# OllieBoyne/sslap

Measured on AMD Instinct MI355X. Metric: Medges/s (bid-phase CSR nnz/s) + solve ms, N=200k d=0.1% sparse LAP, higher is better.
Workload: dtype f64

## Files before the change

sslap_amd/csrc/device_common.hpp:

```cpp
#pragma once
#include <hip/hip_runtime.h>
#include <stdint.h>

#include <type_traits>

namespace misslap {

constexpr int kWave = 64;
constexpr int kPosNone = 0x7fffffff;
constexpr int kTailMax = 512;

#define MISSLAP_KERNEL(BLOCK) MISSLAP_KERNEL_BOUND(BLOCK, BLOCK)
#define MISSLAP_KERNEL_BOUND(BLOCK, BOUND)                                                          \
    static constexpr int kBlock = (BLOCK);    \
    static constexpr int kBound = (BOUND);      \
    static_assert(kBlock <= kBound, "a launch above the kernel's bound fails");                     \
    template <class... A_>                                                                          \
    static __global__ __launch_bounds__(BOUND) void entry(A_... a_) {                               \
        run(a_...);                                                                                 \
    }

constexpr int kErrNegativeBid = 1;
constexpr int kErrRowsUnsorted = 2;
constexpr int kErrRowGap = 4;
// ... 142 lines not shown
};

constexpr int kDppXor1 = 0xB1;
constexpr int kDppXor2 = 0x4E;
constexpr int kDppHalfMirror = 0x141;
constexpr int kDppMirror = 0x140;
constexpr int kDppBcast15 = 0x142;
constexpr int kDppBcast31 = 0x143;
template <int CTRL, int ROW_MASK = 0xF>
__device__ __forceinline__ int dpp_i32(int v) {
    return __builtin_amdgcn_update_dpp(v, v, CTRL, ROW_MASK, 0xF, false);
}
template <int CTRL, int ROW_MASK = 0xF>
__device__ __forceinline__ double dpp_f64(double v) {
    const int lo = dpp_i32<CTRL, ROW_MASK>(__double2loint(v));
    const int hi = dpp_i32<CTRL, ROW_MASK>(__double2hiint(v));
    return __hiloint2double(hi, lo);
}
__device__ __forceinline__ double readlane_f64(double v, int l) {
    const int lo = __builtin_amdgcn_readlane(__double2loint(v), l);
    const int hi = __builtin_amdgcn_readlane(__double2hiint(v), l);
    return __hiloint2double(hi, lo);
}

#define MISSLAP_WAVE_MAX_STEP(T, EXCH) \
    {                                  \
        const T o = EXCH;              \
        v = o > v ? o : v;             \
    }
__device__ __forceinline__ int wave_max_i32(int v) {
    MISSLAP_WAVE_MAX_STEP(int, __builtin_amdgcn_mov_dpp(v, kDppXor1, 0xF, 0xF, true))
    MISSLAP_WAVE_MAX_STEP(int, __builtin_amdgcn_mov_dpp(v, kDppXor2, 0xF, 0xF, true))
    MISSLAP_WAVE_MAX_STEP(int, __builtin_amdgcn_mov_dpp(v, kDppHalfMirror, 0xF, 0xF, true))
    MISSLAP_WAVE_MAX_STEP(int, __builtin_amdgcn_mov_dpp(v, kDppMirror, 0xF, 0xF, true))
    MISSLAP_WAVE_MAX_STEP(int, (dpp_i32<kDppBcast15, 0xA>(v)))
    MISSLAP_WAVE_MAX_STEP(int, (dpp_i32<kDppBcast31, 0xC>(v)))
    return __builtin_amdgcn_readlane(v, 63);
}
__device__ __forceinline__ double wave_max_f64(double v) {
    v = __builtin_fmax(v, dpp_f64<kDppXor1>(v));
    v = __builtin_fmax(v, dpp_f64<kDppXor2>(v));
    v = __builtin_fmax(v, dpp_f64<kDppHalfMirror>(v));
    v = __builtin_fmax(v, dpp_f64<kDppMirror>(v));
    v = __builtin_fmax(v, (dpp_f64<kDppBcast15, 0xA>(v)));
    v = __builtin_fmax(v, (dpp_f64<kDppBcast31, 0xC>(v)));
    return readlane_f64(v, 63);
}
#undef MISSLAP_WAVE_MAX_STEP

struct Top2 {
    double v, w;
    int g;
};
__device__ __forceinline__ Top2 top2_wave_reduce(const Top2 &x) {
    Top2 r;
    r.v = wave_max_f64(x.v);
    r.g = wave_max_i32(x.v == r.v ? x.g : -1);
    r.w = wave_max_f64(x.g == r.g ? x.w : x.v);
    return r;
}

struct __attribute__((aligned(16))) PriceRec {
    double price;
    int owner;
    int ostart;
};

__device__ __forceinline__ int lane_id() { return threadIdx.x & (kWave - 1); }
__device__ __forceinline__ unsigned long long lanemask_lt() {
    return (1ull << lane_id()) - 1ull;
}

constexpr int kCandLanes = 32;
constexpr int kCandMax = 30;
constexpr int kCandMin = 24;
constexpr int kCandRowMax = 4 * kWave;

template <int CTRL>
__device__ __forceinline__ int dppf_i32(int v) {
    return __builtin_amdgcn_mov_dpp(v, CTRL, 0xF, 0xF, true);
}
template <int CTRL>
__device__ __forceinline__ double dppf_f64(double v) {
    return __hiloint2double(dppf_i32<CTRL>(__double2hiint(v)), dppf_i32<CTRL>(__double2loint(v)));
}
__device__ __forceinline__ double half_max_f64(double v) {
    v = __builtin_fmax(v, dppf_f64<kDppXor1>(v));
    v = __builtin_fmax(v, dppf_f64<kDppXor2>(v));
    v = __builtin_fmax(v, dppf_f64<kDppHalfMirror>(v));
    v = __builtin_fmax(v, dppf_f64<kDppMirror>(v));
    v = __builtin_fmax(v, (dpp_f64<kDppBcast15, 0xA>(v)));
    return v;
}
__device__ __forceinline__ int half_max_i32(int v) {
    v = max(v, dppf_i32<kDppXor1>(v));
    v = max(v, dppf_i32<kDppXor2>(v));
    v = max(v, dppf_i32<kDppHalfMirror>(v));
    v = max(v, dppf_i32<kDppMirror>(v));
    v = max(v, (dpp_i32<kDppBcast15, 0xA>(v)));
    return v;
}
__device__ __forceinline__ int half_allmax_i32(int v) {
    v = max(v, dppf_i32<kDppXor1>(v));
    v = max(v, dppf_i32<kDppXor2>(v));
    v = max(v, dppf_i32<kDppHalfMirror>(v));
    v = max(v, dppf_i32<kDppMirror>(v));
    const auto s = __builtin_amdgcn_permlane16_swap(v, v, false, false);
    return max((int)s[0], (int)s[1]);
}

__device__ __forceinline__ double slot_cost(const int2 &s) { return (double)__int_as_float(s.y); }
__device__ __forceinline__ double slot_cost(const Slot64 &s) { return s.c; }
__device__ __forceinline__ double slot_cost_at(const int2 &s, int sl) {
    return (double)__int_as_float(__builtin_amdgcn_readlane(s.y, sl));
}
__device__ __forceinline__ double slot_cost_at(const Slot64 &s, int sl) { return readlane_f64(s.c, sl); }
template <class Slot>
struct LineIO;
template <>
struct LineIO<int2> {
    static __device__ __forceinline__ int2 load(const int2 *cand, const double *, size_t idx) { return cand[idx]; }
    static __device__ __forceinline__ int2 make(int x, int y) { return make_int2(x, y); }
};
template <>
struct LineIO<Slot64> {
    static __device__ __forceinline__ Slot64 load(const int2 *cand, const double *cost, size_t idx) {
        const int2 s = cand[idx];
        Slot64 r;
        r.x = s.x;
        r.y = s.y;
        r.c = cost[idx];
        return r;
    }
    static __device__ __forceinline__ Slot64 make(int x, int y) {
        Slot64 r;
        r.x = x;
        r.y = y;
        r.c = 0.0;
        return r;
    }
};

struct CandBid {
    bool hit;
    unsigned long long key;
    int obj;
    int prev, pstart;
    int len;
};

struct RecSource {
    const PriceRec *rec;
    __device__ __forceinline__ PriceRec get(int col) const { return rec[col]; }
};
struct PriceSource {
    const double *price;
    __device__ __forceinline__ PriceRec get(int col) const {
        PriceRec r;
        r.price = price[col];
        r.owner = -1;
        r.ostart = 0;
        return r;
    }
};

template <class Slot, class Src>
__device__ __forceinline__ PriceRec cand_gather2(const Slot slot, const bool act0, const bool act1, const Src &src) {
    const int lane = lane_id(), l32 = lane & (kCandLanes - 1);
    const bool active = lane < kCandLanes ? act0 : act1;
    const bool is_cand = active & (l32 >= 1) & (l32 <= kCandMax) & (slot.x >= 0);
    return src.get(is_cand ? slot.x : 0);
}
template <class Slot, class Early, class S = NoStamp>
__device__ __forceinline__ void cand_eval2_r(Slot &slot, const PriceRec r, const bool act0, const bool act1,
                                             const double eps, CandBid (&out)[2], int &err, Early &&early,
                                             const S &stamp = S(), int *alive = nullptr);
template <class Slot, class Src, class Early, class S = NoStamp>
__device__ __forceinline__ void cand_eval2(Slot &slot, const bool act0, const bool act1, const Src &src,
                                           const double eps, CandBid (&out)[2], int &err, Early &&early,
                                           const S &stamp = S(), int *alive = nullptr) {
    stamp(1);
    const PriceRec r = cand_gather2(slot, act0, act1, src);
    stamp(2);
    cand_eval2_r(slot, r, act0, act1, eps, out, err, early, stamp, alive);
}
template <class Slot, class Early, class S>
__device__ __forceinline__ void cand_eval2_r(Slot &slot, const PriceRec r, const bool act0, const bool act1,
                                             const double eps, CandBid (&out)[2], int &err, Early &&early,
                                             const S &stamp, int *alive) {
    const int lane = lane_id(), l32 = lane & (kCandLanes - 1);
    const double ninf = -__builtin_huge_val();
    const bool active = lane < kCandLanes ? act0 : act1;
    const bool is_cand = active & (l32 >= 1) & (l32 <= kCandMax) & (slot.x >= 0);
    const double cost = slot_cost(slot);
    double tau[2];
    tau[0] = readlane_f64(__hiloint2double(slot.y, slot.x), 0);
    tau[1] = readlane_f64(__hiloint2double(slot.y, slot.x), kCandLanes);
    out[0].len = __builtin_amdgcn_readlane(slot.x, kCandLanes - 1);
    out[1].len = __builtin_amdgcn_readlane(slot.x, 2 * kCandLanes - 1);
    const double v = is_cand ? cost - r.price : ninf;
    if (alive) {
        const unsigned long long al = __ballot(is_cand & (v >= (lane < kCandLanes ? tau[0] : tau[1])));
        alive[0] = __popc((unsigned)al);
        alive[1] = __popc((unsigned)(al >> 32));
    }
    double V[2], W[2];
    int G[2];
    {
        const double vm = half_max_f64(v);
        V[0] = readlane_f64(vm, 31);
        V[1] = readlane_f64(vm, 63);
        const double Vv = lane < kCandLanes ? V[0] : V[1];
        const int gm = half_max_i32((is_cand & (v == Vv)) ? l32 : -1);
        G[0] = __builtin_amdgcn_readlane(gm, 31);
        G[1] = __builtin_amdgcn_readlane(gm, 63);
    }
    double c1[2];
#pragma unroll
    for (int X = 0; X < 2; ++X) {
        const int sl = kCandLanes * X + max(G[X], 0);
        out[X].obj = __builtin_amdgcn_readlane(slot.x, sl);
        out[X].prev = __builtin_amdgcn_readlane(r.owner, sl);
        out[X].pstart = __builtin_amdgcn_readlane(r.ostart, sl);
        c1[X] = slot_cost_at(slot, sl);
    }
    early(out);
    stamp.light(3);
    const int Gv = lane < kCandLanes ? G[0] : G[1];
    const double wm = half_max_f64(l32 == Gv ? ninf : v);
    W[0] = readlane_f64(wm, 31);
    W[1] = readlane_f64(wm, 63);
#pragma unroll
    for (int X = 0; X < 2; ++X) {
        out[X].hit = (G[X] >= 0) & (V[X] > tau[X]) & (W[X] >= tau[X]);
        const double bid = (c1[X] - W[X]) + eps;
        if (out[X].hit && bid_is_bad(bid)) err |= kErrNegativeBid;
        out[X].key = bid_to_key(bid);
    }
}
template <class Slot, class Src>
__device__ __forceinline__ PriceRec cand_gather1(const Slot &slot, const bool cls, const Src &src) {
    const bool is_cand = cls & (slot.x >= 0);
    return src.get(is_cand ? slot.x : 0);
}
template <class Slot, class Early, class S = NoStamp>
__device__ __forceinline__ void cand_eval1_r(Slot &slot, const PriceRec r, const bool cls, const double eps, CandBid &out,
                                             unsigned &bad_hi, Early &&early, const S &stamp = S());
template <class Slot, class Src, class Early, class S = NoStamp>
__device__ __forceinline__ void cand_eval1(Slot &slot, const bool cls, const Src &src, const double eps, CandBid &out,
                                           unsigned &bad_hi, Early &&early, const S &stamp = S()) {
    stamp(1);
    const PriceRec r = cand_gather1(slot, cls, src);
    stamp(2);
    cand_eval1_r(slot, r, cls, eps, out, bad_hi, early, stamp);
}
template <class Slot, class Early, class S>
__device__ __forceinline__ void cand_eval1_r(Slot &slot, const PriceRec r, const bool cls, const double eps, CandBid &out,
                                             unsigned &bad_hi, Early &&early, const S &stamp) {
    const int lane = lane_id();
    const double ninf = -__builtin_huge_val();
    const bool is_cand = cls & (slot.x >= 0);
    const double cost = slot_cost(slot);
    const double tau = readlane_f64(__hiloint2double(slot.y, slot.x), 0);
    out.len = __builtin_amdgcn_readlane(slot.x, kCandLanes - 1);
    const double v = is_cand ? cost - r.price : ninf;
    const int hi = __double2hiint(v);
    const int k = hi ^ ((hi >> 31) & 0x7fffffff);
    const int km = __builtin_amdgcn_readlane(half_max_i32(k), 31);
    const unsigned eq = (unsigned)(__ballot(k == km) & 0xffffffffull);
    double V;
    int G;
    if (__popc(eq) == 1) {
        G = __ffs((int)eq) - 1;
        V = readlane_f64(v, G);
    } else {
        V = readlane_f64(half_max_f64(v), 31);
        G = __builtin_amdgcn_readlane(half_max_i32((is_cand & (v == V)) ? lane : -1), 31);
    }
    const int sl = max(G, 0);
    out.obj = __builtin_amdgcn_readlane(slot.x, sl);
    out.prev = __builtin_amdgcn_readlane(r.owner, sl);
    out.pstart = __builtin_amdgcn_readlane(r.ostart, sl);
    const double c1 = slot_cost_at(slot, sl);
    early(out);
    stamp.light(3);
    const double W = readlane_f64(half_max_f64(lane == G ? ninf : v), 31);
    out.hit = (G >= 0) & (V > tau) & (W >= tau);
    const double bid = (c1 - W) + eps;
    bad_hi = max(bad_hi, out.hit ? (unsigned)__double2hiint(bid) : 0u);
    out.key = bid_to_key(bid);
}
__device__ __forceinline__ bool bad_hi_is_error(unsigned bad_hi) { return bad_hi > 0x7ff00000u; }
struct NoEarly {
    __device__ __forceinline__ void operator()(const CandBid (&)[2]) const {}
    __device__ __forceinline__ void operator()(const CandBid &) const {}
};

struct CandBuildArgs {
    int c[4];
    double a[4], v[4];
    double V, W;
    int len;
    bool want;
};

__device__ __forceinline__ void cand_build(int2 *cand, double *cost, int person, const CandBuildArgs &ba, double eps,
                                           double &hint) {
    const int lane = lane_id();
    const double ninf = -__builtin_huge_val();
    const int len = ba.len;
    const double W = ba.W;
    unsigned long long okm[4];
#pragma unroll
    for (int u = 0; u < 4; ++u) {
        const int rem = len - kWave * u;
        okm[u] = rem >= kWave ? ~0ull : (rem <= 0 ? 0ull : ((1ull << rem) - 1ull));
    }
    auto count = [&](double t) {
        int n = 0;
#pragma unroll
        for (int u = 0; u < 4; ++u) n += __popcll(__ballot(ba.v[u] >= t) & okm[u]);
        return n;
    };
    double t = ninf;
    int n = len;
    if (len > kCandMax) {
        n = count(W);
        if (n > kCandMax) return;
        t = W;
        double d_ok = 0.0, d_bad = __builtin_huge_val();
        double d = hint > 0.0 ? hint : 4.0 * __builtin_fmax(ba.V - W, eps);
        for (int k = 0; k < 40 && n < kCandMin; ++k) {
            const double t2 = W - d;
            const int n2 = count(t2);
            if (n2 <= kCandMax) {
                d_ok = d;
                t = t2;
                n = n2;
                d = d_bad == __builtin_huge_val() ? 2.0 * d : 0.5 * (d_ok + d_bad);
            } else {
                d_bad = d;
                d = 0.5 * (d_ok + d_bad);
            }
            if (!(d > d_ok) || !(d < d_bad)) break;
        }
        hint = d_ok > 0.0 ? d_ok : hint;
    }
    int2 *line = cand + (size_t)person * kCandLanes;
    int base = 0;
#pragma unroll
    for (int u = 0; u < 4; ++u) {
        const unsigned long long m = __ballot(ba.v[u] >= t) & okm[u];
        if ((m >> lane) & 1ull) {
            const int at = 1 + base + __popcll(m & lanemask_lt());
            line[at] = make_int2(ba.c[u], cost ? 0 : __float_as_int((float)ba.a[u]));
            if (cost) cost[(size_t)person * kCandLanes + at] = ba.a[u];
        }
        base += __popcll(m);
    }
    if (lane < kCandLanes && (lane == 0 || lane == kCandLanes - 1 || lane > n)) {
        int2 x = make_int2(-1, 0);
        if (lane == 0) x = make_int2(__double2loint(t), __double2hiint(t));
        if (lane == kCandLanes - 1) x = make_int2(len, 0);
        line[lane] = x;
    }
}

template <class E, class Src, bool kNT, bool kPre>
__device__ __forceinline__ void wave_bid_full(const E &ed, const Src &src, int s, int e_in,
                                              const typename E::Raw (&pre)[4], double eps, CandBid &out,
                                              CandBuildArgs &ba, int &err) {
    const int lane = lane_id();
    const double ninf = -__builtin_huge_val();
    Top2 x;
    x.v = ninf;
    x.w = ninf;
    x.g = -1;
    int c1 = 0, o1 = -1, os1 = 0;
    double a1 = 0.0;
    int c[4];
    double a[4];
    auto load = [&](int g, int &cc, double &aa) {
        if (kNT) ed.load_nt(g, cc, aa);
        else ed.load(g, cc, aa);
    };
#pragma unroll
    for (int u = 0; u < 4; ++u) {
        if (kPre) E::decode(pre[u], c[u], a[u]);
        else load(s + u * kWave + lane, c[u], a[u]);
    }
    const int e = __builtin_amdgcn_readfirstlane(e_in);
    auto chunk = [&](int base, auto first_) {
        constexpr bool kFirst = decltype(first_)::value;
        PriceRec r[4];
#pragma unroll
        for (int u = 0; u < 4; ++u) {
            const bool ok = base + u * kWave + lane < e;
            if (!ok) c[u] = -1;
            r[u] = src.get(ok ? c[u] : 0);
        }
#pragma unroll
        for (int u = 0; u < 4; ++u) {
            const bool ok = c[u] >= 0;
            const double v = ok ? a[u] - r[u].price : ninf;
            const bool ge = ok & (v >= x.v);
            x.w = __builtin_fmax(x.w, __builtin_fmin(v, x.v));
            x.v = __builtin_fmax(x.v, v);
            x.g = ge ? base + u * kWave + lane : x.g;
            c1 = ge ? c[u] : c1;
            a1 = ge ? a[u] : a1;
            o1 = ge ? r[u].owner : o1;
            os1 = ge ? r[u].ostart : os1;
            if (kFirst && E::kCand) {
                ba.c[u] = c[u];
                ba.a[u] = a[u];
                ba.v[u] = v;
            }
        }
    };
    chunk(s, std::true_type{});
    for (int base = s + 4 * kWave; base < e; base += 4 * kWave) {
#pragma unroll
        for (int u = 0; u < 4; ++u) load(min(base + u * kWave + lane, e - 1), c[u], a[u]);
        chunk(base, std::false_type{});
    }
    const int hi = __double2hiint(x.v);
    const int k = hi ^ ((hi >> 31) & 0x7fffffff);
    const int kmax = wave_max_i32(k);
    const unsigned long long cnd = __ballot(k == kmax);
    int sl;
    double W;
    if (__popcll(cnd) == 1) {
        sl = __ffsll((long long)cnd) - 1;
        W = wave_max_f64(lane == sl ? x.w : x.v);
    } else {
        const int g_mine = x.g;
        const Top2 t2 = top2_wave_reduce(x);
        sl = __ffsll((long long)__ballot(g_mine == t2.g)) - 1;
// ... 134 lines not shown
```

sslap_amd/csrc/kernels_tail.hpp:

```cpp
#pragma once
#include "device_common.hpp"

namespace misslap {

struct TailArgs {
    Ctl *ctl;
    const int *row_ptr;
    double *price;
    PriceRec *rec;
    int *p2o;
    int *o2p;
    int *U;
    int2 *cand;
    double *cand64;
    int thr;
    int round_budget;
    float eps;
};

constexpr int kHashSize = 2048;

__device__ __forceinline__ unsigned long long readlane_u64(unsigned long long v, int l) {
    const int lo = __builtin_amdgcn_readlane((int)(unsigned)(v & 0xffffffffull), l);
    const int hi = __builtin_amdgcn_readlane((int)(unsigned)(v >> 32), l);
    return ((unsigned long long)(unsigned)hi << 32) | (unsigned long long)(unsigned)lo;
}

__device__ __forceinline__ int apply_winner(const TailArgs &a, int person, int pstart, int obj, int prev,
                                            unsigned long long key) {
    PriceRec r;
    r.price = key_to_bid(key);
    r.owner = person;
    r.ostart = pstart;
    a.rec[obj] = r;
    return prev;
}

struct k_sync_from_rec {
    MISSLAP_KERNEL(256)
    static __device__ __forceinline__ void run(Ctl *ctl, const PriceRec *rec, double *price, int *o2p, int *p2o, const int *U, int n_cols, int lines, unsigned long long *live, unsigned ticket) {
        const int K = ctl->K;
        if (blockIdx.x == 0 && threadIdx.x == 0) {
            post_live_status(live, ticket, K, ctl->err, ctl->nits);
            ctl->n_need = 0;
        }
        for (int n = blockIdx.x * blockDim.x + threadIdx.x; n < K; n += gridDim.x * blockDim.x) {
            const int i = U[n];
            if (i >= 0) p2o[i] = -1;
        }
        for (int j = blockIdx.x * blockDim.x + threadIdx.x; j < n_cols; j += gridDim.x * blockDim.x) {
            const PriceRec r = rec[j];
            if (lines && r.price < price[j]) atomicOr(&ctl->err, kErrPriceFell);
            price[j] = r.price;
            o2p[j] = r.owner;
            if (r.owner >= 0) p2o[r.owner] = j;
        }
    }
};


struct TailStats {
    unsigned long long edges, miss_edges, builds;
    unsigned bids, misses;
    unsigned bad_hi;
    int err;
    double hint;
};

__device__ __forceinline__ int lane_zero() {
    return (int)__builtin_amdgcn_mbcnt_hi(0u, __builtin_amdgcn_mbcnt_lo(0u, 0u));
}

template <class Slot>
__device__ __forceinline__ Slot cand_no_line() {
    return (lane_id() & (kCandLanes - 1)) == 0 ? LineIO<Slot>::make(0, 0x7ff00000) : LineIO<Slot>::make(-1, 0);
}
template <class E>
__device__ __forceinline__ typename E::Slot line_of(const TailArgs &a, int p, int l32) {
    return LineIO<typename E::Slot>::load(a.cand, a.cand64, (size_t)max(p, 0) * kCandLanes + l32);
}
template <class E>
struct TwoFetch {
    typename E::Slot slot;
    typename E::Raw row[2][4];
    int ev[2];
};
template <class E>
__device__ __forceinline__ void fetch_row(const TailArgs &a, const E &ed, int person, int start,
                                          typename E::Raw (&row)[4], int &e) {
    const int lane = lane_id();
#pragma unroll
    for (int u = 0; u < 4; ++u) row[u] = ed.load_raw_nt(start + u * kWave + lane);
    e = a.row_ptr[max(person, 0) + 1 + lane_zero()];
}
template <class E>
__device__ __forceinline__ void request_two(const TailArgs &a, const E &ed, int p0, int s0, int p1, int s1,
                                            TwoFetch<E> &tf) {
    if (E::kCand) {
        const int pme = lane_id() < kCandLanes ? p0 : p1;
        tf.slot = a.cand != nullptr ? line_of<E>(a, pme, lane_id() & (kCandLanes - 1)) : cand_no_line<typename E::Slot>();
    } else {
        fetch_row<E>(a, ed, p0, s0, tf.row[0], tf.ev[0]);
        fetch_row<E>(a, ed, p1, s1, tf.row[1], tf.ev[1]);
    }
}

__device__ __forceinline__ void tail_build(const TailArgs &a, int person, const CandBuildArgs &ba, double eps,
                                           TailStats &st) {
    cand_build(a.cand, a.cand64, person, ba, eps, st.hint);
    st.builds += 1;
}

template <class E, class Early, class S = NoStamp>
__device__ __forceinline__ void bid_two(const TailArgs &a, const E &ed, const int (&pi)[2], const int (&ps)[2],
                                        TwoFetch<E> &tf, double eps, CandBid (&b)[2], CandBuildArgs &bd,
                                        int &bd_person, TailStats &st, Early &&early, const S &stamp = S()) {
    const RecSource src{a.rec};
    b[0].hit = b[1].hit = false;
    if (E::kCand) cand_eval2(tf.slot, pi[0] >= 0, pi[1] >= 0, src, eps, b, st.err, early, stamp);
    stamp.light(4);
    bd_person = -1;
#pragma unroll
    for (int X = 0; X < 2; ++X) {
        if (pi[X] < 0) continue;
        if (!b[X].hit) {
            if (bd_person >= 0) tail_build(a, bd_person, bd, eps, st);
            if (E::kCand) {
                const typename E::Raw none[4] = {};
                const int e = a.row_ptr[pi[X] + 1 + lane_zero()];
                wave_bid_full<E, RecSource, true, false>(ed, src, ps[X], e, none, eps, b[X], bd, st.err);
            } else {
                wave_bid_full<E, RecSource, true, true>(ed, src, ps[X], tf.ev[X], tf.row[X], eps, b[X], bd, st.err);
            }
            bd.want = bd.want && a.cand != nullptr;
            bd_person = bd.want ? pi[X] : -1;
            st.misses += 1;
            st.miss_edges += (unsigned long long)b[X].len;
        }
        st.edges += (unsigned long long)b[X].len;
        st.bids += 1;
    }
}

__device__ __forceinline__ int round_limit(long long nits, long long max_iter) {
    return (int)min(max_iter - nits, (long long)0x7fffffff);
}

template <class E>
__device__ __forceinline__ void tail_chain_mode(const TailArgs &a, const E &ed, int &pi, int &ps, int &K,
                                                long long &nits, const long long max_iter, const double eps,
                                                TailStats &st) {
    const int lane = lane_id(), l32 = lane & (kCandLanes - 1);
    const RecSource src{a.rec};
    const bool cls = (lane >= 1) & (lane <= kCandMax);
    const bool lines = E::kCand && a.cand != nullptr;
    typename E::Slot slot = cand_no_line<typename E::Slot>();
    typename E::Raw row[4];
    int ev = 0;
    auto request = [&](int person, int start) {
        if (E::kCand) {
            if (lines) slot = line_of<E>(a, person, l32);
        } else {
            fetch_row<E>(a, ed, person, start, row, ev);
        }
    };
    request(pi, ps);
    const int rmax = round_limit(nits, max_iter);
    int r = 0;
#ifdef MISSLAP_TAIL_STAMP
    unsigned long long sacc[8] = {0, 0, 0, 0, 0, 0, 0, 0}, sprev = __builtin_amdgcn_s_memtime();
    const CycleStamp stamp{sacc, &sprev, true};
#else
    const NoStamp stamp;
#endif
    for (;;) {
        CandBid b;
        b.hit = false;
        int sp = -2;
        if (E::kCand)
            cand_eval1(slot, cls, src, eps, b, st.bad_hi, [&](const CandBid &w) {
                sp = w.prev;
                request(sp, 0);
            }, stamp);
        stamp.light(4);
        if (!b.hit) {
            CandBuildArgs bd;
            if (E::kCand) {
                const typename E::Raw none[4] = {};
                const int e = a.row_ptr[pi + 1];
                wave_bid_full<E, RecSource, true, false>(ed, src, ps, e, none, eps, b, bd, st.err);
            } else {
                wave_bid_full<E, RecSource, true, true>(ed, src, ps, ev, row, eps, b, bd, st.err);
            }
            st.misses += 1;
            st.miss_edges += (unsigned long long)b.len;
            if (bd.want && lines) tail_build(a, pi, bd, eps, st);
        }
        stamp.light(5);
        st.edges += (unsigned long long)b.len;
        st.bids += 1;
        r += 1;
        if (lane == 0) apply_winner(a, pi, ps, b.obj, b.prev, b.key);
        pi = b.prev;
        ps = b.pstart;
        const bool done = pi < 0 || r >= rmax;
        if (!done && sp != pi) request(pi, ps);
        stamp.light(6);
        if (done) break;
    }
    K = pi != -1;
    nits += r;
#ifdef MISSLAP_TAIL_STAMP
    if (lane == 0) {
        for (int k = 1; k <= 6; ++k) a.ctl->dbg[5 + k] += sacc[k];
    }
#endif
}

template <class E>
__device__ __forceinline__ void tail_solo_mode(const TailArgs &a, const E &ed, int *sU, int *sStart, int &K,
                                               long long &nits, const long long max_iter, const double eps,
                                               TailStats &st) {
    const int lane = lane_id();
    int pi[2], ps[2];
    pi[0] = __builtin_amdgcn_readfirstlane(sU[0]);
    ps[0] = __builtin_amdgcn_readfirstlane(sStart[0]);
    pi[1] = K > 1 ? __builtin_amdgcn_readfirstlane(sU[1]) : -1;
    ps[1] = K > 1 ? __builtin_amdgcn_readfirstlane(sStart[1]) : 0;
    if (K == 1) {
        tail_chain_mode(a, ed, pi[0], ps[0], K, nits, max_iter, eps, st);
        if (lane == 0) {
            sU[0] = pi[0];
            sU[1] = -1;
            sStart[0] = ps[0];
        }
        return;
    }
    TwoFetch<E> tf;
    tf.slot = cand_no_line<typename E::Slot>();
    request_two(a, ed, pi[0], ps[0], pi[1], ps[1], tf);
#ifdef MISSLAP_TAIL_STAMP_SOLO
    unsigned long long sacc[8] = {0, 0, 0, 0, 0, 0, 0, 0}, sprev = __builtin_amdgcn_s_memtime();
    const CycleStamp stamp{sacc, &sprev, true};
#else
    const NoStamp stamp;
#endif
    for (;;) {
        CandBid b[2];
        CandBuildArgs bd;
        int bd_person;
        int sp[2] = {-2, -2};
        bid_two(a, ed, pi, ps, tf, eps, b, bd, bd_person, st, [&](const CandBid(&w)[2]) {
            sp[0] = pi[0] >= 0 ? w[0].prev : -1;
            sp[1] = pi[1] >= 0 ? w[1].prev : -1;
            request_two(a, ed, sp[0], 0, sp[1], 0, tf);
        }, stamp);
        stamp.light(5);
        nits += 1;
        bool win0 = true, win1 = pi[1] >= 0;
        if (win1 && b[0].obj == b[1].obj) {
            if (b[1].key > b[0].key) win0 = false;
            else win1 = false;
        }
        if (lane == 0) {
            if (win0) apply_winner(a, pi[0], ps[0], b[0].obj, b[0].prev, b[0].key);
            if (win1) apply_winner(a, pi[1], ps[1], b[1].obj, b[1].prev, b[1].key);
        }
        if (win0) {
            pi[0] = b[0].prev;
            ps[0] = b[0].pstart;
        }
        if (win1) {
            pi[1] = b[1].prev;
            ps[1] = b[1].pstart;
        }
        if (pi[0] == -1 && pi[1] != -1) {
            pi[0] = pi[1];
            ps[0] = ps[1];
            pi[1] = -1;
        }
        K = (pi[0] != -1) + (pi[1] != -1);
        const bool done = K <= 1 || nits >= max_iter;
        if (!done && (sp[0] != pi[0] || sp[1] != pi[1])) request_two(a, ed, pi[0], ps[0], pi[1], ps[1], tf);
        if (bd_person >= 0) tail_build(a, bd_person, bd, eps, st);
        stamp.light(6);
        if (done) break;
    }
    if (K == 1 && nits < max_iter) tail_chain_mode(a, ed, pi[0], ps[0], K, nits, max_iter, eps, st);
#ifdef MISSLAP_TAIL_STAMP_SOLO
    if (lane == 0)
        for (int k = 1; k <= 6; ++k) a.ctl->dbg[5 + k] += sacc[k];
#endif
    if (lane == 0) {
        sU[0] = pi[0];
        sU[1] = pi[1];
        sStart[0] = ps[0];
        sStart[1] = ps[1];
    }
}

template <class E>
__device__ __forceinline__ void tail_pair_mode(const TailArgs &a, const E &ed, int *sU, int *sStart, int &K,
                                               long long &nits, const long long max_iter, const double eps,
                                               TailStats &st) {
    const int lane = lane_id(), l32 = lane & (kCandLanes - 1);
    const bool upper = lane >= kCandLanes;
    const RecSource src{a.rec};
    const bool cls = (l32 >= 1) & (l32 <= kCandMax);
    const double ninf = -__builtin_huge_val();
    int pi[2], ps[2];
#pragma unroll
    for (int X = 0; X < 2; ++X) {
        pi[X] = __builtin_amdgcn_readfirstlane(sU[X]);
        ps[X] = __builtin_amdgcn_readfirstlane(sStart[X]);
    }
    typename E::Slot slot;
    auto request = [&](int p0, int p1) { slot = line_of<E>(a, upper ? p1 : p0, l32); };
    const int rmax = round_limit(nits, max_iter);
    int r = 0;
    if (K == 2) request(pi[0], pi[1]);
#ifdef MISSLAP_TAIL_STAMP_DUO
    unsigned long long sacc[8] = {0, 0, 0, 0, 0, 0, 0, 0}, sprev = __builtin_amdgcn_s_memtime();
    const CycleStamp stamp{sacc, &sprev, true};
#else
    const NoStamp stamp;
#endif
    while (K == 2) {
        stamp(1);
        const PriceRec g = cand_gather1(slot, cls, src);
        stamp(2);
        const bool is_cand = cls & (slot.x >= 0);
        const double v = is_cand ? slot_cost(slot) - g.price : ninf;
        const int hw = __double2hiint(v);
        const int k = hw ^ ((hw >> 31) & 0x7fffffff);
        const unsigned long long eq = __ballot(k == half_allmax_i32(k));
        const unsigned eq0 = (unsigned)eq, eq1 = (unsigned)(eq >> 32);
        int G[2];
        double V[2];
        if ((int)(__popc(eq0) == 1) & (int)(__popc(eq1) == 1)) {
            G[0] = __ffs((int)eq0) - 1;
            G[1] = __ffs((int)eq1) + (kCandLanes - 1);
            V[0] = readlane_f64(v, G[0]);
            V[1] = readlane_f64(v, G[1]);
        } else {
            const double vm = half_max_f64(v);
            V[0] = readlane_f64(vm, kCandLanes - 1);
            V[1] = readlane_f64(vm, kWave - 1);
            const int gm = half_max_i32((is_cand & (v == (upper ? V[1] : V[0]))) ? lane : -1);
            G[0] = __builtin_amdgcn_readlane(gm, kCandLanes - 1);
            G[1] = __builtin_amdgcn_readlane(gm, kWave - 1);
        }
        CandBid b[2];
        double tau[2], c1[2];
#pragma unroll
        for (int X = 0; X < 2; ++X) {
            const int sl = max(G[X], kCandLanes * X);
            tau[X] = readlane_f64(__hiloint2double(slot.y, slot.x), kCandLanes * X);
            b[X].len = __builtin_amdgcn_readlane(slot.x, kCandLanes * X + kCandLanes - 1);
            b[X].obj = __builtin_amdgcn_readlane(slot.x, sl);
            b[X].prev = __builtin_amdgcn_readlane(g.owner, sl);
            b[X].pstart = __builtin_amdgcn_readlane(g.ostart, sl);
            c1[X] = slot_cost_at(slot, sl);
        }
        const int sp0 = b[0].prev, sp1 = b[1].prev;
        request(sp0, sp1);
        stamp.light(3);
        const double wm = half_max_f64(((lane == G[0]) | (lane == G[1])) ? ninf : v);
        const double W[2] = {readlane_f64(wm, kCandLanes - 1), readlane_f64(wm, kWave - 1)};
#pragma unroll
        for (int X = 0; X < 2; ++X) {
            b[X].hit = (G[X] >= 0) & (V[X] > tau[X]) & (W[X] >= tau[X]);
            const double bid = (c1[X] - W[X]) + eps;
            st.bad_hi = max(st.bad_hi, b[X].hit ? (unsigned)__double2hiint(bid) : 0u);
            b[X].key = bid_to_key(bid);
        }
        stamp.light(4);
#pragma unroll
        for (int X = 0; X < 2; ++X) {
            if (!b[X].hit) {
                CandBuildArgs bd;
                const typename E::Raw none[4] = {};
                const int e = a.row_ptr[pi[X] + 1];
                wave_bid_full<E, RecSource, true, false>(ed, src, ps[X], e, none, eps, b[X], bd, st.err);
                st.misses += 1;
                st.miss_edges += (unsigned long long)b[X].len;
                if (bd.want) tail_build(a, pi[X], bd, eps, st);
            }
        }
        stamp.light(5);
        st.edges += (unsigned long long)(b[0].len + b[1].len);
        st.bids += 2;
        r += 1;
        if ((b[0].obj != b[1].obj) & (b[0].prev >= 0) & (b[1].prev >= 0)) {
            if (l32 == 0) {
                PriceRec w;
                w.price = key_to_bid(upper ? b[1].key : b[0].key);
                w.owner = upper ? pi[1] : pi[0];
                w.ostart = upper ? ps[1] : ps[0];
                a.rec[upper ? b[1].obj : b[0].obj] = w;
            }
#pragma unroll
            for (int X = 0; X < 2; ++X) {
                pi[X] = b[X].prev;
                ps[X] = b[X].pstart;
            }
        } else {
            bool win0 = true, win1 = true;
            if (b[0].obj == b[1].obj) {
                if (b[1].key > b[0].key) win0 = false;
                else win1 = false;
            }
            if (lane == 0) {
                if (win0) apply_winner(a, pi[0], ps[0], b[0].obj, b[0].prev, b[0].key);
                if (win1) apply_winner(a, pi[1], ps[1], b[1].obj, b[1].prev, b[1].key);
            }
            if (win0) {
                pi[0] = b[0].prev;
                ps[0] = b[0].pstart;
            }
            if (win1) {
                pi[1] = b[1].prev;
                ps[1] = b[1].pstart;
            }
            if (pi[0] == -1 && pi[1] != -1) {
                pi[0] = pi[1];
                ps[0] = ps[1];
                pi[1] = -1;
            }
            K = (pi[0] != -1) + (pi[1] != -1);
        }
        const bool done = K <= 1 || r >= rmax;
        if (!done && (sp0 != pi[0] || sp1 != pi[1])) request(pi[0], pi[1]);
        stamp.light(6);
        if (done) break;
    }
    nits += r;
#ifdef MISSLAP_TAIL_STAMP_DUO
    if (lane == 0)
        for (int k = 1; k <= 6; ++k) a.ctl->dbg[5 + k] += sacc[k];
#endif
    if (K == 1 && nits < max_iter) tail_chain_mode(a, ed, pi[0], ps[0], K, nits, max_iter, eps, st);
    if (lane == 0) {
        sU[0] = pi[0];
        sU[1] = pi[1];
        sStart[0] = ps[0];
        sStart[1] = ps[1];
    }
}

constexpr int kTeamMax = 16;
constexpr int kTeamTab = 64;
__device__ __forceinline__ void tail_barrier_lds() { asm volatile("s_waitcnt lgkmcnt(0)\n\ts_barrier" ::: "memory"); }

template <class E>
__device__ __forceinline__ void tail_team_mode(const TailArgs &a, const E &ed, int *sU, int *sStart, int &K,
                                               long long &nits, const long long max_iter, const double eps,
                                               TailStats &st) {
    const int lane = lane_id(), wave = __builtin_amdgcn_readfirstlane(threadIdx.x >> 6);
    static_assert(kTeamMax <= 2 * (kTailMax / kWave) && kTeamMax <= kWave, "two list slots per wavefront");
    __shared__ unsigned long long tKey[2][kTeamMax];
    __shared__ int tObj[2][kTeamMax], tPrev[2][kTeamMax], tPst[2][kTeamMax], tU[2][kTeamMax], tS[2][kTeamMax];
    __shared__ int wTab[kTailMax / kWave][kTeamTab];
    const int n0 = 2 * wave;
    int pi[2], ps[2];
#pragma unroll
    for (int X = 0; X < 2; ++X) {
        pi[X] = n0 + X < K ? __builtin_amdgcn_readfirstlane(sU[min(n0 + X, kTailMax - 1)]) : -1;
        ps[X] = n0 + X < K ? __builtin_amdgcn_readfirstlane(sStart[min(n0 + X, kTailMax - 1)]) : 0;
    }
    wTab[wave][lane & (kTeamTab - 1)] = -1;
    TwoFetch<E> tf;
    tf.slot = cand_no_line<typename E::Slot>();
    if (n0 < K) request_two(a, ed, pi[0], ps[0], pi[1], ps[1], tf);
    __syncthreads();
#ifdef MISSLAP_TAIL_STAMP_TEAM
    unsigned long long sacc[8] = {0, 0, 0, 0, 0, 0, 0, 0}, sprev = __builtin_amdgcn_s_memtime();
    const CycleStamp stamp{sacc, &sprev, wave == 0};
#else
    const NoStamp stamp;
#endif
    int par = 0;
    for (;;) {
        int sp[2] = {-2, -2};
        CandBuildArgs bd;
        int bd_person = -1;
        stamp.light(0);
        if (n0 < K) {
            CandBid b[2];
            bid_two(a, ed, pi, ps, tf, eps, b, bd, bd_person, st, [&](const CandBid(&w)[2]) {
                sp[0] = pi[0] >= 0 ? w[0].prev : -1;
                sp[1] = pi[1] >= 0 ? w[1].prev : -1;
                request_two(a, ed, sp[0], 0, sp[1], 0, tf);
            });
            if (lane == 0) {
#pragma unroll
                for (int X = 0; X < 2; ++X)
                    if (pi[X] >= 0) {
                        tKey[par][n0 + X] = b[X].key;
                        tObj[par][n0 + X] = b[X].obj;
                        tPrev[par][n0 + X] = b[X].prev;
                        tPst[par][n0 + X] = b[X].pstart;
                        tU[par][n0 + X] = pi[X];
                        tS[par][n0 + X] = ps[X];
                    }
            }
        }
        stamp.light(1);
        tail_barrier_lds();
        stamp.light(2);
        {
            const bool act = lane < K;
            const int ls = min(lane, kTeamMax - 1);
            const unsigned long long lkey = act ? tKey[par][ls] : 0ull;
            const int lobj = act ? tObj[par][ls] : (-2 - lane);
            const int lprev = act ? tPrev[par][ls] : 0, lpst = act ? tPst[par][ls] : 0;
            int u = act ? tU[par][ls] : -1;
            int sx = act ? tS[par][ls] : 0;
            int hs = 0;
            bool dup = false;
            if (act) {
                hs = (int)(((unsigned)lobj * 2654435761u) >> 26) & (kTeamTab - 1);
                for (;;) {
                    const int old = atomicCAS(&wTab[wave][hs], -1, lobj);
                    if (old == -1) break;
                    if (old == lobj) {
                        dup = true;
                        break;
                    }
                    hs = (hs + 1) & (kTeamTab - 1);
                }
            }
            const bool contested = __any(dup);
            if (act && !dup) wTab[wave][hs] = -1;
            const bool ends = __any(act && lprev == -1);
#ifdef MISSLAP_TAIL_STAMP_TEAM
            if (threadIdx.x == 0) sacc[5] += (!contested && !ends), sacc[6] += contested, sacc[7] += 1;
#endif
            if (!contested && !ends) {
                if (act && n0 < K) apply_winner(a, u, sx, lobj, lprev, lkey);
#pragma unroll
                for (int X = 0; X < 2; ++X) {
                    const int w = __builtin_amdgcn_readlane(lprev, min(n0 + X, kWave - 1));
                    const int ws = __builtin_amdgcn_readlane(lpst, min(n0 + X, kWave - 1));
                    pi[X] = n0 + X < K ? w : -1;
                    ps[X] = n0 + X < K ? ws : 0;
                }
            } else {
                bool lose = false;
                for (int m = 0; m < K; ++m) {
                    const int om = __builtin_amdgcn_readlane(lobj, m);
                    const bool same = (om == lobj) && (m != lane);
                    if (__any(same)) {
                        const unsigned long long km = readlane_u64(lkey, m);
                        lose |= same && (km > lkey || (km == lkey && m < lane));
                    }
                }
                const bool won = act && !lose;
                if (won && n0 < K) apply_winner(a, u, sx, lobj, lprev, lkey);
                u = won ? lprev : u;
                sx = won ? lpst : sx;
                const unsigned long long kmask = (1ull << K) - 1ull;
                const unsigned long long holes = __ballot(act && u == -1) & kmask;
                const int Kn = K - __popcll(holes);
                const unsigned long long lmask = (1ull << Kn) - 1ull;
                unsigned long long hl = holes & lmask;
                unsigned long long mv = ~holes & ~lmask & kmask;
                while (hl) {
                    const int hk = __ffsll((long long)hl) - 1, mk = __ffsll((long long)mv) - 1;
                    const int mu = __builtin_amdgcn_readlane(u, mk), ms = __builtin_amdgcn_readlane(sx, mk);
                    if (lane == hk) {
                        u = mu;
                        sx = ms;
                    }
                    hl &= hl - 1;
                    mv &= mv - 1;
                }
                K = Kn;
#pragma unroll
                for (int X = 0; X < 2; ++X) {
                    pi[X] = n0 + X < K ? __builtin_amdgcn_readlane(u, min(n0 + X, kWave - 1)) : -1;
                    ps[X] = n0 + X < K ? __builtin_amdgcn_readlane(sx, min(n0 + X, kWave - 1)) : 0;
                }
            }
        }
        stamp.light(3);
        par ^= 1;
        nits += 1;
// ... 578 lines not shown
```

Baseline: 4831.

## Issue next candidate-line prefetch from high-word argmax and double-buffer tail slots

In the single-chain and duo tail loops, the owner of the best candidate is now found from the high 32 bits of the bid value alone. That lets the next person's candidate line be requested before the full f64 argmax and second-best reductions run. Candidate slots are double-buffered (slotA/slotB, with the loop unrolled by two) so the prefetch writes a separate register set while the current one is still in use. The gather now uses an unsigned, masked index, and sched_barriers pin the ordering. The prefetch is speculative: on a high-word tie or a mismatch the line is fetched again, which costs an extra load and adds register pressure.

```diff
diff --git a/sslap_amd/csrc/device_common.hpp b/sslap_amd/csrc/device_common.hpp
--- a/sslap_amd/csrc/device_common.hpp
+++ b/sslap_amd/csrc/device_common.hpp
@@ -318,6 +318,7 @@
 struct RecSource {
     const PriceRec *rec;
     __device__ __forceinline__ PriceRec get(int col) const { return rec[col]; }
+    __device__ __forceinline__ PriceRec get_u(unsigned col) const { return rec[(size_t)col]; }
 };
 struct PriceSource {
     const double *price;
@@ -412,14 +413,6 @@
 template <class Slot, class Early, class S = NoStamp>
 __device__ __forceinline__ void cand_eval1_r(Slot &slot, const PriceRec r, const bool cls, const double eps, CandBid &out,
                                              unsigned &bad_hi, Early &&early, const S &stamp = S());
-template <class Slot, class Src, class Early, class S = NoStamp>
-__device__ __forceinline__ void cand_eval1(Slot &slot, const bool cls, const Src &src, const double eps, CandBid &out,
-                                           unsigned &bad_hi, Early &&early, const S &stamp = S()) {
-    stamp(1);
-    const PriceRec r = cand_gather1(slot, cls, src);
-    stamp(2);
-    cand_eval1_r(slot, r, cls, eps, out, bad_hi, early, stamp);
-}
 template <class Slot, class Early, class S>
 __device__ __forceinline__ void cand_eval1_r(Slot &slot, const PriceRec r, const bool cls, const double eps, CandBid &out,
                                              unsigned &bad_hi, Early &&early, const S &stamp) {
@@ -450,6 +443,61 @@
     const double c1 = slot_cost_at(slot, sl);
     early(out);
     stamp.light(3);
+    const double W = readlane_f64(half_max_f64(lane == G ? ninf : v), 31);
+    out.hit = (G >= 0) & (V > tau) & (W >= tau);
+    const double bid = (c1 - W) + eps;
+    bad_hi = max(bad_hi, out.hit ? (unsigned)__double2hiint(bid) : 0u);
+    out.key = bid_to_key(bid);
+}
+template <class Slot, class Src>
+__device__ __forceinline__ PriceRec cand_gather1_u(const Slot &slot, const bool cls, const Src &src) {
+    const int keep = cls ? 0x7fffffff : 0;
+    return src.get_u((unsigned)(max(slot.x, 0) & keep));
+}
+template <class Slot, class Early, class S = NoStamp>
+__device__ __forceinline__ void cand_eval1_front_r(const Slot &slot, const PriceRec r, const bool cls, const double eps,
+                                                   CandBid &out, unsigned &bad_hi, Early &&early, const S &stamp = S());
+template <class Slot, class Src, class Early, class S = NoStamp>
+__device__ __forceinline__ void cand_eval1_front(const Slot &slot, const bool cls, const Src &src, const double eps,
+                                                 CandBid &out, unsigned &bad_hi, Early &&early, const S &stamp = S()) {
+    stamp(1);
+    const PriceRec r = cand_gather1_u(slot, cls, src);
+    stamp(2);
+    cand_eval1_front_r(slot, r, cls, eps, out, bad_hi, early, stamp);
+}
+template <class Slot, class Early, class S>
+__device__ __forceinline__ void cand_eval1_front_r(const Slot &slot, const PriceRec r, const bool cls, const double eps,
+                                                   CandBid &out, unsigned &bad_hi, Early &&early, const S &stamp) {
+    const int lane = lane_id();
+    const double ninf = -__builtin_huge_val();
+    const bool is_cand = cls & (slot.x >= 0);
+    const double cost = slot_cost(slot);
+    const double tau = readlane_f64(__hiloint2double(slot.y, slot.x), 0);
+    out.len = __builtin_amdgcn_readlane(slot.x, kCandLanes - 1);
+    __builtin_amdgcn_sched_barrier(0);
+    const double d = cost - r.price;
+    const int hi = is_cand ? __double2hiint(d) : __double2hiint(ninf);
+    const int k = hi ^ ((hi >> 31) & 0x7fffffff);
+    const unsigned eq = (unsigned)(__ballot(k == half_allmax_i32(k)) & 0xffffffffull);
+    const int Gp = __builtin_ctz(eq);
+    early(__builtin_amdgcn_readlane(r.owner, Gp));
+    __builtin_amdgcn_sched_barrier(0);
+    stamp.light(3);
+    const double v = __hiloint2double(hi, is_cand ? __double2loint(d) : 0);
+    double V;
+    int G;
+    if (__popc(eq) == 1) {
+        G = Gp;
+        V = readlane_f64(v, G);
+    } else {
+        V = readlane_f64(half_max_f64(v), 31);
+        G = __builtin_amdgcn_readlane(half_max_i32((is_cand & (v == V)) ? lane : -1), 31);
+    }
+    const int sl = max(G, 0);
+    out.obj = __builtin_amdgcn_readlane(slot.x, sl);
+    out.prev = __builtin_amdgcn_readlane(r.owner, sl);
+    out.pstart = __builtin_amdgcn_readlane(r.ostart, sl);
+    const double c1 = slot_cost_at(slot, sl);
     const double W = readlane_f64(half_max_f64(lane == G ? ninf : v), 31);
     out.hit = (G >= 0) & (V > tau) & (W >= tau);
     const double bid = (c1 - W) + eps;
diff --git a/sslap_amd/csrc/kernels_tail.hpp b/sslap_amd/csrc/kernels_tail.hpp
--- a/sslap_amd/csrc/kernels_tail.hpp
+++ b/sslap_amd/csrc/kernels_tail.hpp
@@ -154,17 +154,17 @@
     const RecSource src{a.rec};
     const bool cls = (lane >= 1) & (lane <= kCandMax);
     const bool lines = E::kCand && a.cand != nullptr;
-    typename E::Slot slot = cand_no_line<typename E::Slot>();
+    typename E::Slot slotA = cand_no_line<typename E::Slot>(), slotB = slotA;
     typename E::Raw row[4];
     int ev = 0;
-    auto request = [&](int person, int start) {
+    auto request = [&](typename E::Slot &dst, int person, int start) {
         if (E::kCand) {
-            if (lines) slot = line_of<E>(a, person, l32);
+            if (lines) dst = line_of<E>(a, person, l32);
         } else {
             fetch_row<E>(a, ed, person, start, row, ev);
         }
     };
-    request(pi, ps);
+    request(slotA, pi, ps);
     const int rmax = round_limit(nits, max_iter);
     int r = 0;
 #ifdef MISSLAP_TAIL_STAMP
@@ -173,14 +173,14 @@
 #else
     const NoStamp stamp;
 #endif
-    for (;;) {
+    auto round = [&](const typename E::Slot &cur, typename E::Slot &nxt) -> bool {
         CandBid b;
         b.hit = false;
         int sp = -2;
         if (E::kCand)
-            cand_eval1(slot, cls, src, eps, b, st.bad_hi, [&](const CandBid &w) {
-                sp = w.prev;
-                request(sp, 0);
+            cand_eval1_front(cur, cls, src, eps, b, st.bad_hi, [&](int owner) {
+                sp = owner;
+                request(nxt, sp, 0);
             }, stamp);
         stamp.light(4);
         if (!b.hit) {
@@ -204,9 +204,13 @@
         pi = b.prev;
         ps = b.pstart;
         const bool done = pi < 0 || r >= rmax;
-        if (!done && sp != pi) request(pi, ps);
+        if (!done && sp != pi) request(nxt, pi, ps);
         stamp.light(6);
-        if (done) break;
+        return done;
+    };
+    for (;;) {
+        if (round(slotA, slotB)) break;
+        if (round(slotB, slotA)) break;
     }
     K = pi != -1;
     nits += r;
@@ -314,32 +318,47 @@
         pi[X] = __builtin_amdgcn_readfirstlane(sU[X]);
         ps[X] = __builtin_amdgcn_readfirstlane(sStart[X]);
     }
-    typename E::Slot slot;
-    auto request = [&](int p0, int p1) { slot = line_of<E>(a, upper ? p1 : p0, l32); };
+    typename E::Slot slotA = cand_no_line<typename E::Slot>(), slotB = slotA;
+    auto request = [&](typename E::Slot &dst, int p0, int p1) { dst = line_of<E>(a, upper ? p1 : p0, l32); };
     const int rmax = round_limit(nits, max_iter);
     int r = 0;
-    if (K == 2) request(pi[0], pi[1]);
+    if (K == 2) request(slotA, pi[0], pi[1]);
 #ifdef MISSLAP_TAIL_STAMP_DUO
     unsigned long long sacc[8] = {0, 0, 0, 0, 0, 0, 0, 0}, sprev = __builtin_amdgcn_s_memtime();
     const CycleStamp stamp{sacc, &sprev, true};
 #else
     const NoStamp stamp;
 #endif
-    while (K == 2) {
+    auto round = [&](const typename E::Slot &slot, typename E::Slot &nxt) -> bool {
         stamp(1);
-        const PriceRec g = cand_gather1(slot, cls, src);
+        const PriceRec g = cand_gather1_u(slot, cls, src);
+        const bool is_cand = cls & (slot.x >= 0);
+        const double cost = slot_cost(slot);
+        CandBid b[2];
+        double tau[2];
+#pragma unroll
+        for (int X = 0; X < 2; ++X) {
+            tau[X] = readlane_f64(__hiloint2double(slot.y, slot.x), kCandLanes * X);
+            b[X].len = __builtin_amdgcn_readlane(slot.x, kCandLanes * X + kCandLanes - 1);
+        }
+        __builtin_amdgcn_sched_barrier(0);
         stamp(2);
-        const bool is_cand = cls & (slot.x >= 0);
-        const double v = is_cand ? slot_cost(slot) - g.price : ninf;
-        const int hw = __double2hiint(v);
+        const double d = cost - g.price;
+        const int hw = is_cand ? __double2hiint(d) : __double2hiint(ninf);
         const int k = hw ^ ((hw >> 31) & 0x7fffffff);
         const unsigned long long eq = __ballot(k == half_allmax_i32(k));
         const unsigned eq0 = (unsigned)eq, eq1 = (unsigned)(eq >> 32);
+        const int Gp0 = __builtin_ctz(eq0), Gp1 = __builtin_ctz(eq1) + kCandLanes;
+        const int sp0 = __builtin_amdgcn_readlane(g.owner, Gp0), sp1 = __builtin_amdgcn_readlane(g.owner, Gp1);
+        request(nxt, sp0, sp1);
+        __builtin_amdgcn_sched_barrier(0);
+        stamp.light(3);
+        const double v = __hiloint2double(hw, is_cand ? __double2loint(d) : 0);
         int G[2];
         double V[2];
         if ((int)(__popc(eq0) == 1) & (int)(__popc(eq1) == 1)) {
-            G[0] = __ffs((int)eq0) - 1;
-            G[1] = __ffs((int)eq1) + (kCandLanes - 1);
+            G[0] = Gp0;
+            G[1] = Gp1;
             V[0] = readlane_f64(v, G[0]);
             V[1] = readlane_f64(v, G[1]);
         } else {
@@ -350,21 +369,15 @@
             G[0] = __builtin_amdgcn_readlane(gm, kCandLanes - 1);
             G[1] = __builtin_amdgcn_readlane(gm, kWave - 1);
         }
-        CandBid b[2];
-        double tau[2], c1[2];
+        double c1[2];
 #pragma unroll
         for (int X = 0; X < 2; ++X) {
             const int sl = max(G[X], kCandLanes * X);
-            tau[X] = readlane_f64(__hiloint2double(slot.y, slot.x), kCandLanes * X);
-            b[X].len = __builtin_amdgcn_readlane(slot.x, kCandLanes * X + kCandLanes - 1);
             b[X].obj = __builtin_amdgcn_readlane(slot.x, sl);
             b[X].prev = __builtin_amdgcn_readlane(g.owner, sl);
             b[X].pstart = __builtin_amdgcn_readlane(g.ostart, sl);
             c1[X] = slot_cost_at(slot, sl);
         }
-        const int sp0 = b[0].prev, sp1 = b[1].prev;
-        request(sp0, sp1);
-        stamp.light(3);
         const double wm = half_max_f64(((lane == G[0]) | (lane == G[1])) ? ninf : v);
         const double W[2] = {readlane_f64(wm, kCandLanes - 1), readlane_f64(wm, kWave - 1)};
 #pragma unroll
@@ -430,9 +443,13 @@
             K = (pi[0] != -1) + (pi[1] != -1);
         }
         const bool done = K <= 1 || r >= rmax;
-        if (!done && (sp0 != pi[0] || sp1 != pi[1])) request(pi[0], pi[1]);
+        if (!done && (sp0 != pi[0] || sp1 != pi[1])) request(nxt, pi[0], pi[1]);
         stamp.light(6);
-        if (done) break;
+        return done;
+    };
+    while (K == 2) {
+        if (round(slotA, slotB)) break;
+        if (round(slotB, slotA)) break;
     }
     nits += r;
 #ifdef MISSLAP_TAIL_STAMP_DUO
```

Result: no change. 4878, median of 6 (+1.0%).
